# gmlwns2000/sea-attention

Measured on AMD Instinct MI355X. Metric: tokens/sec + achieved HBM GB/s, OPT-1.3B SEA T=4096 k=64, 1/2/4/8 MI355X, higher is better.
Workload: dtype bf16

## Files before the change

sea-attention_amd/csrc/sea_topk.hip:

```cpp
#include "sea_common.hpp"
#include "sea_tail.hpp"
#include "sea_convfrag.hpp"


#ifdef SEA_STAMP
__device__ unsigned long long sea_dbg[16];
#define STAMP(i) do { if (threadIdx.x == 0) { unsigned long long _t = __builtin_amdgcn_s_memtime(); \
  atomicAdd(&sea_dbg[i], _t - _tprev); _tprev = _t; } } while (0)
#else
#define STAMP(i) do {} while (0)
#endif

namespace sea {

constexpr int TK_THREADS = 256;
constexpr int TK_WAVES = TK_THREADS / WAVE;
constexpr int TK_MAX_BINS = 2048;

__device__ inline uint32_t f2key(float f) {
  f = f + 0.0f;
  uint32_t u = __float_as_uint(f);
  return u ^ ((u >> 31) ? 0xFFFFFFFFu : 0x80000000u);
}

struct TopkParams {
  const void* src;
  int64_t sn, sh, st;
  int H, T_dst, T_m, T_src;
  int is_causal, max_k;
  int M;
  int nchunks;
  int W;
  int G;
  const int32_t* keep;
  int64_t keep_stride_n;
  uint32_t* bits;
  float* mask_out;
  int32_t* row_nnz;
  int32_t* head_off;
  const int32_t* t_src_dev;
  int t_src_stride;
  int32_t* crow1;
};

template <typename T> __device__ inline void load4(const T* p, float* f);
template <> __device__ inline void load4<float>(const float* p, float* f) {
  float4 v = *reinterpret_cast<const float4*>(p);
  f[0] = v.x; f[1] = v.y; f[2] = v.z; f[3] = v.w;
}
template <> __device__ inline void load4<__hip_bfloat16>(const __hip_bfloat16* p, float* f) {
  uint2 v = *reinterpret_cast<const uint2*>(p);
  f[0] = __uint_as_float(v.x << 16); f[1] = __uint_as_float(v.x & 0xffff0000u);
  f[2] = __uint_as_float(v.y << 16); f[3] = __uint_as_float(v.y & 0xffff0000u);
}
template <> __device__ inline void load4<__half>(const __half* p, float* f) {
  uint2 v = *reinterpret_cast<const uint2*>(p);
  const __half2* h = reinterpret_cast<const __half2*>(&v);
  float2 a = __half22float2(h[0]), b = __half22float2(h[1]);
  f[0] = a.x; f[1] = a.y; f[2] = b.x; f[3] = b.y;
}

__device__ inline int block_excl_scan(int v, int* s_wave , int* total) {
  const int lane = threadIdx.x & 63, w = threadIdx.x >> 6;
  int incl = wave_incl_scan(v);
  if (lane == 63) s_wave[w] = incl;
  __syncthreads();
  int base = 0, tot = 0;
#pragma unroll
  for (int i = 0; i < TK_WAVES; ++i) {
    int x = s_wave[i];
    if (i < w) base += x;
    tot += x;
  }
  __syncthreads();
  *total = tot;
  return base + incl - v;
}

template <typename T>
__device__ __noinline__ unsigned long long select_multipass(const T* base, int64_t sh, int T_m, int nchunks, int M, int K,
                                                            uint32_t umin, uint32_t umax, int rounds, int* s_hist,
                                                            int* s_wave, int* s_bcast) {
  const int tid = threadIdx.x;
  auto load_keys = [&](int j, uint32_t* k4) -> bool {
    const int c = j * TK_THREADS + tid;
    if (c >= nchunks) { k4[0] = k4[1] = k4[2] = k4[3] = 0u; return false; }
    const int f0 = c * 4;
    const int h = f0 / T_m, b0 = f0 - h * T_m;
    float f[4];
    load4<T>(base + h * sh + b0, f);
    for (int e = 0; e < 4; ++e) k4[e] = f2key(f[e]);
    return true;
  };
  unsigned long long sel = 0;
  uint32_t prefix = umax;
  int bits_left = (umax == umin) ? 0 : (32 - __clz(umax ^ umin));
  int kth = K, n_eq = M;
  while (bits_left > 0) {
    const int d = bits_left < 11 ? bits_left : 11;
    const int shift = bits_left - d;
    const int nb = 1 << d;
    const int hi = shift + d;
    for (int i = tid; i < nb; i += TK_THREADS) s_hist[i] = 0;
    __syncthreads();
    for (int j = 0; j < rounds; ++j) {
      uint32_t k4[4];
      if (!load_keys(j, k4)) continue;
      for (int e = 0; e < 4; ++e) {
        const uint32_t u = k4[e];
        const bool cand = (hi >= 32) ? true : ((u >> hi) == (prefix >> hi));
        if (cand) atomicAdd(&s_hist[nb - 1 - (int)((u >> shift) & (uint32_t)(nb - 1))], 1);
      }
    }
    __syncthreads();
    const int per = (nb + TK_THREADS - 1) / TK_THREADS;
    int mine = 0;
    for (int i = 0; i < per; ++i) {
      const int bi = tid * per + i;
      if (bi < nb) mine += s_hist[bi];
    }
    int total;
    const int excl = block_excl_scan(mine, s_wave, &total);
    if (excl < kth && kth <= excl + mine) {
      int run = excl;
      for (int i = 0; i < per; ++i) {
        const int bi = tid * per + i;
        const int c = s_hist[bi];
        if (kth <= run + c) { s_bcast[0] = bi; s_bcast[1] = run; s_bcast[2] = c; break; }
        run += c;
      }
    }
    __syncthreads();
    const int rb = s_bcast[0];
    kth -= s_bcast[1];
    n_eq = s_bcast[2];
    const uint32_t dmask = (uint32_t)(nb - 1) << shift;
    prefix = (prefix & ~dmask) | ((uint32_t)(nb - 1 - rb) << shift);
    bits_left = shift;
    __syncthreads();
  }
  const uint32_t tau = prefix;
  const int r = kth;
  int seen = 0;
  for (int j = 0; j < rounds; ++j) {
    uint32_t k4[4];
    const bool valid = load_keys(j, k4);
    int cnt = 0;
    for (int e = 0; e < 4; ++e) cnt += (valid && k4[e] == tau) ? 1 : 0;
    int total = 0, rank = 0;
    if (n_eq != r) rank = seen + block_excl_scan(cnt, s_wave, &total);
    for (int e = 0; e < 4; ++e) {
      if (!valid) continue;
      if (k4[e] > tau) sel |= 1ull << (4 * j + e);
      if (k4[e] == tau) {
        if (n_eq == r || rank < r) sel |= 1ull << (4 * j + e);
        ++rank;
      }
    }
    seen += total;
  }
  return sel;
}

__device__ inline long long block_excl_scan64(long long v, long long* s_wave , long long* total) {
  const int lane = threadIdx.x & 63, w = threadIdx.x >> 6;
  long long incl = wave_incl_scan(v);
  if (lane == 63) s_wave[w] = incl;
  __syncthreads();
  long long base = 0, tot = 0;
#pragma unroll
  for (int i = 0; i < TK_WAVES; ++i) {
    const long long x = s_wave[i];
    if (i < w) base += x;
    tot += x;
  }
  __syncthreads();
  *total = tot;
  return base + incl - v;
}

template <typename T, int EPT, bool FROM_MASK, bool FULL, int HMAX = 1024, bool EXT_CAND = false, bool K16 = false, bool HCW = K16>
__device__ __forceinline__ void select_body(const TopkParams& p, uint32_t (&key)[K16 ? EPT / 2 : EPT], unsigned long long sel, int n,
                                            int t, int row, const T* base, uint32_t* cand = nullptr) {
  constexpr int R = EPT / 4;
  static_assert(!K16 || (sizeof(T) == 2 && !FROM_MASK), "packed keys: 16-bit maps");
  auto key_at = [&](int i) -> uint32_t {
    if constexpr (K16) return (i & 1) ? (key[i >> 1] >> 16) : (key[i >> 1] & 0xffffu);
    else return key[i];
  };
  auto digit_at = [&](int i, int shift, int d) -> int {
    if constexpr (K16) return (int)__builtin_amdgcn_ubfe(~key[i >> 1], shift + 16 * (i & 1), d);
    else return (int)__builtin_amdgcn_ubfe(~key[i], shift, d);
  };
  __shared__ int s_hist[TK_MAX_BINS + 1];
  __shared__ int s_head[HMAX];
  __shared__ int s_wave[TK_WAVES];
  __shared__ uint32_t s_red[2 * TK_WAVES];
  __shared__ int s_bcast[4];
  uint32_t* s_ckey;
  uint32_t* s_cidx;
  if constexpr (EXT_CAND) {
    s_ckey = cand; s_cidx = cand + TK_CAND_CAP;
  } else {
    __shared__ uint32_t s_cand[2 * TK_CAND_CAP];
    s_ckey = s_cand; s_cidx = s_cand + TK_CAND_CAP;
  }
  __shared__ uint32_t s_selbits[512];
  __shared__ int s_ncand;

  const int tid = threadIdx.x;
  const int lane = tid & 63, wv = tid >> 6;
#ifdef SEA_STAMP
  unsigned long long _tprev = __builtin_amdgcn_s_memtime();
#endif
  for (int i = tid; i <= TK_MAX_BINS; i += TK_THREADS) s_hist[i] = 0;
  for (int i = tid; i < 512; i += TK_THREADS) s_selbits[i] = 0;
  for (int i = tid; i < p.H; i += TK_THREADS) s_head[i] = 0;
  if (tid == 0) s_ncand = 0;

  if (!FROM_MASK) {
    const int K = p.keep[n * p.keep_stride_n + t + (p.t_src_dev ? p.t_src_dev[n * p.t_src_stride] - p.T_dst : 0)];
    if (K >= p.M) {
#pragma unroll
      for (int j = 0; j < R; ++j)
        if (FULL || j * TK_THREADS + tid < p.nchunks) sel |= 0xFull << (4 * j);
      __syncthreads();
    } else if (K <= 0) {
      __syncthreads();
    } else {
      uint32_t umin = 0xFFFFFFFFu, umax = 0u;
      if constexpr (K16) {
        typedef unsigned short us2 __attribute__((ext_vector_type(2)));
        us2 mn = us2{0xFFFF, 0xFFFF}, mx = us2{0, 0};
#pragma unroll
        for (int j = 0; j < R; ++j) {
          if (FULL || j * TK_THREADS + tid < p.nchunks) {
            const us2 a = __builtin_bit_cast(us2, key[2 * j]), b = __builtin_bit_cast(us2, key[2 * j + 1]);
            mn = __builtin_elementwise_min(mn, __builtin_elementwise_min(a, b));
            mx = __builtin_elementwise_max(mx, __builtin_elementwise_max(a, b));
          }
        }
        umin = min((uint32_t)mn[0], (uint32_t)mn[1]);
        umax = max((uint32_t)mx[0], (uint32_t)mx[1]);
      } else {
#pragma unroll
      for (int j = 0; j < R; ++j) {
        if (FULL || j * TK_THREADS + tid < p.nchunks) {
          umin = min(umin, min(min(key[4 * j], key[4 * j + 1]), min(key[4 * j + 2], key[4 * j + 3])));
          umax = max(umax, max(max(key[4 * j], key[4 * j + 1]), max(key[4 * j + 2], key[4 * j + 3])));
        }
      }
      }
      umin = wave_min(umin);
      umax = wave_max(umax);
      if (lane == 0) { s_red[wv] = umin; s_red[TK_WAVES + wv] = umax; }
      __syncthreads();
#pragma unroll
      for (int i = 0; i < TK_WAVES; ++i) { umin = min(umin, s_red[i]); umax = max(umax, s_red[TK_WAVES + i]); }
      STAMP(1);
      const int bits_left = (umax == umin) ? 0 : (32 - __clz(umax ^ umin));
      bool fast = bits_left > 0;
      int rb_sel = 0, kth = K, c_in = 0, shift = 0, d = 0;
      if (fast) {
        d = bits_left < 11 ? bits_left : 11;
        shift = bits_left - d;
        const int nb = 1 << d;
#pragma unroll
        for (int i = 0; i < EPT; ++i) {
          int rb = digit_at(i, shift, d);
          if (!FULL) rb = (((i >> 2) * TK_THREADS + tid) < p.nchunks) ? rb : TK_MAX_BINS;
          atomicAdd(&s_hist[rb], 1);
        }
        __syncthreads();
        const int per = (nb + TK_THREADS - 1) / TK_THREADS;
        int mine = 0;
        for (int i = 0; i < per; ++i) {
          const int bi = tid * per + i;
          if (bi < nb) mine += s_hist[bi];
        }
        int total;
        const int excl = block_excl_scan(mine, s_wave, &total);
        if (excl < K && K <= excl + mine) {
          int run = excl;
          for (int i = 0; i < per; ++i) {
            const int bi = tid * per + i;
            const int c = s_hist[bi];
            if (K <= run + c) { s_bcast[0] = bi; s_bcast[1] = run; s_bcast[2] = c; break; }
            run += c;
          }
        }
        __syncthreads();
        rb_sel = s_bcast[0];
        kth = K - s_bcast[1];
        c_in = s_bcast[2];
        fast = c_in <= TK_CAND_CAP;
      }
      STAMP(2);
      if (fast) {
#pragma unroll
        for (int i = 0; i < EPT; ++i) {
          const int rb = digit_at(i, shift, d);
          const bool valid = FULL || (((i >> 2) * TK_THREADS + tid) < p.nchunks);
          if (valid && rb < rb_sel) sel |= 1ull << i;
          if (valid && rb == rb_sel) {
            const int slot = atomicAdd(&s_ncand, 1);
            s_ckey[slot] = key_at(i);
            s_cidx[slot] = (uint32_t)(((i >> 2) * TK_THREADS + tid) * 4 + (i & 3));
          }
        }
        __syncthreads();
        for (int ci = tid; ci < c_in; ci += TK_THREADS) {
          const uint32_t ku = s_ckey[ci], kf = s_cidx[ci];
          int rank = 0;
          for (int cj = 0; cj < c_in; ++cj) {
            const uint32_t ou = s_ckey[cj], of = s_cidx[cj];
            rank += (ou > ku || (ou == ku && of < kf)) ? 1 : 0;
          }
          if (rank < kth) atomicOr(&s_selbits[kf >> 5], 1u << (kf & 31));
        }
        __syncthreads();
#pragma unroll
        for (int j = 0; j < R; ++j) {
          const int c = j * TK_THREADS + tid;
          const unsigned long long nibx = (s_selbits[(c >> 3) & 511] >> (4 * (c & 7))) & 0xFu;
          sel |= nibx << (4 * j);
        }
      } else if constexpr (K16) {
        const bool hist = bits_left > 0;
        int n_eq = hist ? c_in : p.M;
        uint32_t tau_low = 0u;
        const uint32_t lowmask = hist ? ((1u << shift) - 1u) : 0u;
        auto in_bin = [&](int i) -> bool {
          const bool valid = FULL || (((i >> 2) * TK_THREADS + tid) < p.nchunks);
          return valid && (!hist || digit_at(i, shift, d) == rb_sel);
        };
        if (hist) {
#pragma unroll
          for (int i = 0; i < EPT; ++i) {
            const bool valid = FULL || (((i >> 2) * TK_THREADS + tid) < p.nchunks);
            if (valid && digit_at(i, shift, d) < rb_sel) sel |= 1ull << i;
          }
          if (shift > 0) {
            const int nb2 = 1 << shift;
            __syncthreads();
            if (tid < nb2) s_hist[tid] = 0;
            __syncthreads();
#pragma unroll
            for (int i = 0; i < EPT; ++i)
              if (in_bin(i)) atomicAdd(&s_hist[nb2 - 1 - (int)(key_at(i) & lowmask)], 1);
            __syncthreads();
            const int mine = tid < nb2 ? s_hist[tid] : 0;
            int total;
            const int excl = block_excl_scan(mine, s_wave, &total);
            if (tid < nb2 && excl < kth && kth <= excl + mine) { s_bcast[0] = tid; s_bcast[1] = excl; s_bcast[2] = mine; }
            __syncthreads();
            tau_low = (uint32_t)(nb2 - 1 - s_bcast[0]);
            kth -= s_bcast[1];
            n_eq = s_bcast[2];
#pragma unroll
            for (int i = 0; i < EPT; ++i)
              if (in_bin(i) && (key_at(i) & lowmask) > tau_low) sel |= 1ull << i;
          }
        }
        int seen = 0;
#pragma unroll
        for (int j = 0; j < R; ++j) {
          bool tie[4];
          int cnt = 0;
#pragma unroll
          for (int e = 0; e < 4; ++e) {
            tie[e] = in_bin(4 * j + e) && (key_at(4 * j + e) & lowmask) == tau_low;
            cnt += tie[e] ? 1 : 0;
          }
          int total = 0, rank = 0;
          if (n_eq != kth) rank = seen + block_excl_scan(cnt, s_wave, &total);
#pragma unroll
          for (int e = 0; e < 4; ++e) {
            if (tie[e]) {
              if (n_eq == kth || rank < kth) sel |= 1ull << (4 * j + e);
              ++rank;
            }
          }
          seen += total;
        }
        __syncthreads();
      } else {
        sel = select_multipass<T>(base, p.sh, p.T_m, p.nchunks, p.M, K, umin, umax, R, s_hist, s_wave, s_bcast);
        for (int i = tid; i < p.H; i += TK_THREADS) s_head[i] = 0;
        __syncthreads();
      }
    }
  } else {
    __syncthreads();
  }

  STAMP(3);
  const int w_t = row_width(t, p.T_dst, p.t_src_dev ? p.t_src_dev[n * p.t_src_stride] : p.T_src, p.is_causal);
  const float scale = interp_scale(w_t, p.T_m);
  const bool tm_pow2 = (p.T_m & (p.T_m - 1)) == 0;
  const int tm_sh = __ffs(p.T_m) - 1;
#pragma unroll
  for (int j = 0; j < R; ++j) {
    const int c = j * TK_THREADS + tid;
    const bool valid = FULL || c < p.nchunks;
    const uint32_t nib = (uint32_t)(sel >> (4 * j)) & 0xFu;
    uint32_t word = nib << (4 * (lane & 7));
    word |= dpp_u32<0xB1>(word);
    word |= dpp_u32<0x4E>(word);
    word |= dpp_u32<0x141>(word);
    if ((lane & 7) == 0 && (c >> 3) < p.W) p.bits[(int64_t)row * p.W + (c >> 3)] = word;
    if (p.mask_out != nullptr && valid) {
      const int f0 = c * 4;
      const int h = f0 / p.T_m, b0 = f0 - h * p.T_m;
      float4 m;
      m.x = (nib & 1u) ? 1.f : 0.f; m.y = (nib & 2u) ? 1.f : 0.f;
      m.z = (nib & 4u) ? 1.f : 0.f; m.w = (nib & 8u) ? 1.f : 0.f;
      *reinterpret_cast<float4*>(p.mask_out + (((int64_t)n * p.H + h) * p.T_dst + t) * p.T_m + b0) = m;
    }
  }
  if constexpr (K16 && HCW) {
    int wpx[4];
    {
      float bprev = interp_bound(4 * lane, scale);
#pragma unroll
      for (int e = 0; e < 4; ++e) {
        const float bnext = interp_bound(4 * lane + e + 1, scale);
        const int w = (int)(bnext - bprev);
        wpx[e] = w < p.max_k ? w : p.max_k;
        bprev = bnext;
      }
    }
#pragma unroll
    for (int j0 = 0; j0 < R; j0 += 8) {
      float red[8];
#pragma unroll
      for (int b = 0; b < 8; ++b) {
        int sum = 0;
        if (j0 + b < R) {
          const uint32_t nib = (uint32_t)(sel >> (4 * (j0 + b))) & 0xFu;
#pragma unroll
          for (int e = 0; e < 4; ++e) sum += (nib >> e) & 1u ? wpx[e] : 0;
        }
        red[b] = (float)sum;
      }
      const float x = wave_reduce8(red, [](float u, float v) { return u + v; });
#pragma unroll
      for (int b = 0; b < 8; ++b) {
        const int h = 4 * (j0 + b) + wv;
        if (j0 + b < R && h < p.H && lane == 0) s_head[h] = (int)reduce8_get(x, b);
      }
    }
  } else {
    unsigned long long m = sel;
    while (m) {
      const int i = __ffsll((long long)m) - 1;
      m &= m - 1;
      const int f = ((i >> 2) * TK_THREADS + tid) * 4 + (i & 3);
      const int h = tm_pow2 ? (f >> tm_sh) : f / p.T_m, b = f - h * p.T_m;
      int w = (int)(interp_bound(b + 1, scale) - interp_bound(b, scale));
      w = w < p.max_k ? w : p.max_k;
      if (w > 0) atomicAdd(&s_head[h], w);
    }
  }
  __syncthreads();
  STAMP(4);
  if (wv == 0) {
    int carry = 0;
    int32_t* ho = p.head_off + (int64_t)row * (p.H + 1);
    for (int h0 = 0; h0 < p.H; h0 += 64) {
      const int h = h0 + lane;
      const int v = h < p.H ? s_head[h] : 0;
      const int incl = wave_incl_scan(v);
      if (h < p.H) ho[h] = carry + incl - v;
      carry += __shfl(incl, 63);
    }
    if (lane == 0) {
      ho[p.H] = carry; p.row_nnz[row] = carry;
      if (p.crow1 != nullptr) { p.crow1[2 * row] = 0; p.crow1[2 * row + 1] = carry; }
    }
  }
}

template <typename T, int EPT, bool FROM_MASK, bool FULL>
__global__ __launch_bounds__(TK_THREADS) void topk_select_kernel(TopkParams p) {
  constexpr int R = EPT / 4;
  const int tid = threadIdx.x;
  const int row = blockIdx.x;
  const int n = row / p.T_dst, t = row - n * p.T_dst;
  const T* base = reinterpret_cast<const T*>(p.src) + n * p.sn + t * p.st;
#ifdef SEA_STAMP
  unsigned long long _tprev = __builtin_amdgcn_s_memtime();
#endif

  uint32_t key[EPT];
  unsigned long long sel = 0;
#pragma unroll
  for (int j = 0; j < R; ++j) {
    const int c = j * TK_THREADS + tid;
    float f[4] = {0.f, 0.f, 0.f, 0.f};
    const bool valid = FULL || c < p.nchunks;
    if (valid) {
      const int f0 = c * 4;
      const int h = f0 / p.T_m, b0 = f0 - h * p.T_m;
      load4<T>(base + h * p.sh + b0, f);
    }
#pragma unroll
    for (int e = 0; e < 4; ++e) {
      if (FROM_MASK) {
        if (valid && f[e] != 0.f) sel |= 1ull << (4 * j + e);
        key[4 * j + e] = 0;
      } else {
        key[4 * j + e] = valid ? f2key(f[e]) : 0u;
      }
    }
  }
  STAMP(0);
  select_body<T, EPT, FROM_MASK, FULL>(p, key, sel, n, t, row, base);
}

template <typename T, int EPT, bool FULL>
__device__ __forceinline__ void tail_select_row(const TailParams& tp, const TopkParams& p, float* s_z, int row) {
#include "sea_tail_select_row.inc"
}

template <typename T, int EPT, bool FULL>
#ifndef SEA_TSEL_OCC32
#define SEA_TSEL_OCC32 7
#endif
#ifndef SEA_TSEL_OCC16
#define SEA_TSEL_OCC16 7
#endif
__global__ __launch_bounds__(TK_THREADS, EPT <= 16 ? SEA_TSEL_OCC16 : EPT == 32 ? SEA_TSEL_OCC32 : EPT == 40 ? 5 : 1) void predictor_tail_select_kernel(TailParams tp, TopkParams p) {
  extern __shared__ __attribute__((aligned(16))) float s_z[];
  const int row = blockIdx.x;
#include "sea_tail_select_row.inc"
}

template <int EPT>
__global__ __launch_bounds__(TK_THREADS) void predictor_tail_select_f32_kernel(TailParams tp, TopkParams p) {
  using T = float;
  constexpr bool FULL = false;
  static_assert(EPT <= 32, "one batch of eight heads per wave (H <= 32)");
  extern __shared__ __attribute__((aligned(16))) float s_z[];
  const int row = blockIdx.x;
#include "sea_tail_select_row.inc"
}

template <typename T, int E, int EPT>
__device__ __forceinline__ void tail_select_row_gen(const TailParams& tp, const TopkParams& p, float* s_z, int row) {
  constexpr bool TAB_LDS = false;
#include "sea_tail_select_row_gen.inc"
}

template <typename T, int E, int EPT>
__global__ __launch_bounds__(TK_THREADS) void predictor_tail_select_gen_kernel(TailParams tp, TopkParams p) {
  constexpr bool TAB_LDS = true;
  extern __shared__ __attribute__((aligned(16))) float s_z[];
  const int row = blockIdx.x;
#include "sea_tail_select_row_gen.inc"
}

template <typename I>
__global__ __launch_bounds__(1024) void row_scan_kernel(const int32_t* row_nnz, int T_dst, I* crow) {
  constexpr int PER = 16;
  __shared__ int s_w[2][16];
  const int n = blockIdx.x;
  const int tid = threadIdx.x, lane = tid & 63, w = tid >> 6;
  const int32_t* src = row_nnz + (int64_t)n * T_dst;
  I* dst = crow + (int64_t)n * (T_dst + 1);
  long long carry = 0;
  for (int t0 = 0; t0 < T_dst; t0 += 1024 * PER) {
    int vv[PER];
#pragma unroll
    for (int j = 0; j < PER; ++j) {
      const int t = t0 + j * 1024 + tid;
      vv[j] = t < T_dst ? src[t] : 0;
    }
#pragma unroll
    for (int j = 0; j < PER; ++j) {
      if (t0 + j * 1024 < T_dst) {
        const int t = t0 + j * 1024 + tid;
        const int v = vv[j];
        const int incl = wave_incl_scan(v);
        if (lane == 63) s_w[j & 1][w] = incl;
        __syncthreads();
        int base = 0, tot = 0;
#pragma unroll
        for (int i = 0; i < 16; ++i) { const int x = s_w[j & 1][i]; if (i < w) base += x; tot += x; }
        if (t < T_dst) dst[t] = (I)(carry + base + incl - v);
        carry += tot;
      }
    }
    __syncthreads();
  }
  if (tid == 0) dst[T_dst] = (I)carry;
}

struct EmitParams {
  const uint32_t* bits;
  const void* crow;
  int H, T_dst, T_m, T_src, is_causal, max_k, W;
  void* col;
  int64_t col_stride_n, z_cap;
  float* values_out;
  int T_enc;
  const int32_t* t_src_dev;
  int t_src_stride;
};

constexpr int EM_TABLE = 1024;
constexpr int EM_WIN = 4096;

template <typename I>
__device__ __forceinline__ void csr_emit_row(const EmitParams& p, const int row) {
  __shared__ int s_wave[TK_WAVES];
  __shared__ int s_bound[EM_TABLE + 1];
  __shared__ int s_out[EM_WIN];
  const int tid = threadIdx.x;
  const int n = row / p.T_dst, t = row - n * p.T_dst;
  const I* crow = reinterpret_cast<const I*>(p.crow) + (int64_t)n * (p.T_dst + 1);
  const int64_t row_beg = (int64_t)crow[t];
  const int64_t row_end = (int64_t)crow[t + 1];
  if (row_end == row_beg) return;
  I* col = reinterpret_cast<I*>(p.col) + n * p.col_stride_n;
  float* vals = p.values_out ? p.values_out + n * p.col_stride_n : nullptr;
  const uint32_t* bits = p.bits + (int64_t)row * p.W;
  const int w_t = row_width(t, p.T_dst, p.t_src_dev ? p.t_src_dev[n * p.t_src_stride] : p.T_src, p.is_causal);
  const float scale = interp_scale(w_t, p.T_m);
  const bool table = p.T_m <= EM_TABLE;
  if (table)
    for (int m = tid; m <= p.T_m; m += TK_THREADS) s_bound[m] = (int)interp_bound(m, scale);
  __syncthreads();
  auto bnd = [&](int m) { return table ? s_bound[m] : (int)interp_bound(m, scale); };
  const bool aligned = (p.T_m & 31) == 0;
  const bool direct = sizeof(I) == 4 && vals == nullptr && aligned && w_t >= 4 * p.T_m && (w_t + p.T_m - 1) / p.T_m <= p.max_k;

  int carry = 0;
  for (int w0 = 0; w0 < p.W; w0 += TK_THREADS) {
    const int wi = w0 + tid;
    uint32_t word = wi < p.W ? bits[wi] : 0u;
    const int f0 = wi * 32;
    const int h0 = f0 / p.T_m, b0 = f0 - h0 * p.T_m;
    int nent = 0;
    if (direct) {
      const int npmax = __builtin_amdgcn_readfirstlane(wave_max(__popc(word)));
      uint32_t m = word;
      for (int it = 0; it < npmax; ++it) {
        const bool act = m != 0u;
        const int b = b0 + (act ? __ffs(m) - 1 : 0);
        m &= m - 1;
        const int wd = bnd(b + 1) - bnd(b);
        nent += act ? wd : 0;
      }
    } else {
      for (uint32_t m = word; m;) {
        const int bit = __ffs(m) - 1;
        m &= m - 1;
        int b = b0 + bit;
        if (!aligned) b %= p.T_m;
        const int wd = bnd(b + 1) - bnd(b);
        nent += wd < p.max_k ? wd : p.max_k;
      }
    }
    int total;
    const int excl = block_excl_scan(nent, s_wave, &total);
    if (direct) {
      const int wlo = w_t / p.T_m;
      const int nst = (wlo + 1 + 3) >> 2;
      const int npmax = __builtin_amdgcn_readfirstlane(wave_max(__popc(word)));
      int64_t off = row_beg + carry + excl;
      uint32_t m = word;
      const int hb = h0 * p.T_enc;
      for (int it = 0; it < npmax; ++it) {
        const bool act = m != 0u;
        const int bit = act ? __ffs(m) - 1 : 0;
        m &= m - 1;
        const int b = b0 + bit;
        const int lo = bnd(b), hi = bnd(b + 1);
        const int wd = hi - lo;
        if (act && off + wd <= p.z_cap) {
          int32_t* dst = reinterpret_cast<int32_t*>(col) + off;
          const int c0 = hb + hi - 1;
          typedef int ei4 __attribute__((ext_vector_type(4), aligned(4)));
          for (int i = 0; i < nst; ++i) {
            const int j = min(4 * i, wd - 4);
            const int c = c0 - j;
            const ei4 v = {c, c - 1, c - 2, c - 3};
            *reinterpret_cast<ei4*>(dst + j) = v;
          }
        }
        off += act ? wd : 0;
      }
      carry += total;
      continue;
    }
    for (int win = (carry / EM_WIN) * EM_WIN; win < carry + total; win += EM_WIN) {
      int off = carry + excl;
      if (nent > 0 && off < win + EM_WIN && off + nent > win) {
        const bool inside = off >= win && off + nent <= win + EM_WIN;
        for (uint32_t m = word; m;) {
          const int bit = __ffs(m) - 1;
          m &= m - 1;
          int h = h0, b = b0 + bit;
          if (!aligned) { const int q = b / p.T_m; h += q; b -= q * p.T_m; }
          const int lo = bnd(b), hi = bnd(b + 1);
          const int wd = hi - lo;
          const int hb = h * p.T_enc;
          if (wd <= p.max_k) {
            if (inside) {
              int* dst = s_out + (off - win);
              const int c0 = hb + hi - 1;
              for (int j = 0; j < wd; ++j) dst[j] = c0 - j;
            } else {
              for (int j = 0; j < wd; ++j) {
                const int o = off + j - win;
                if ((unsigned)o < (unsigned)EM_WIN) s_out[o] = hb + hi - 1 - j;
              }
            }
            off += wd;
          } else {
// ... 661 lines not shown
```

Before: 16.30 million.

## Classify top-k candidates with scalar key-range compares and wave-aggregated slot allocation

The fast top-k path used to extract a radix digit per element and take one shared-memory atomicAdd for each candidate. It now compares each key against a wave-uniform key range held in SGPRs using inline v_cmp/v_addc asm, which builds 'above' and 'candidate' bitmasks directly. It then reserves candidate slots with one atomic per wave via a wave prefix scan, and uses a binary select tree to read keys out of the register array. The bitmask store loop is also split so all words are computed first and stored afterwards. The inline asm and the key-range derivation from umax add correctness risk across edge cases.

```diff
diff --git a/sea-attention_amd/csrc/sea_topk.hip b/sea-attention_amd/csrc/sea_topk.hip
--- a/sea-attention_amd/csrc/sea_topk.hip
+++ b/sea-attention_amd/csrc/sea_topk.hip
@@ -179,6 +179,23 @@
   return base + incl - v;
 }
 
+__device__ __forceinline__ void shift_in_gt_ge(uint32_t& a, uint32_t& b, uint32_t top, uint32_t lo, uint32_t x) {
+  asm("v_cmp_lt_u32_e32 vcc, %2, %4\n\tv_addc_co_u32_e32 %0, vcc, %0, %0, vcc\n\t"
+      "v_cmp_le_u32_e32 vcc, %3, %4\n\tv_addc_co_u32_e32 %1, vcc, %1, %1, vcc"
+      : "+v"(a), "+v"(b) : "s"(top), "s"(lo), "v"(x) : "vcc");
+}
+
+template <int LO, int N, int NK> __device__ __forceinline__ uint32_t pick_reg(const uint32_t (&a)[NK], int r) {
+  static_assert(N >= 1 && LO + N <= NK, "inside the array");
+  if constexpr (N == 1) {
+    return a[LO];
+  } else {
+    constexpr int HALF = 1 << (31 - __builtin_clz((unsigned)(N - 1)));
+    const uint32_t lo = pick_reg<LO, HALF>(a, r), hi = pick_reg<LO + HALF, N - HALF>(a, r);
+    return (r & HALF) ? hi : lo;
+  }
+}
+
 template <typename T, int EPT, bool FROM_MASK, bool FULL, int HMAX = 1024, bool EXT_CAND = false, bool K16 = false, bool HCW = K16>
 __device__ __forceinline__ void select_body(const TopkParams& p, uint32_t (&key)[K16 ? EPT / 2 : EPT], unsigned long long sel, int n,
                                             int t, int row, const T* base, uint32_t* cand = nullptr) {
@@ -297,17 +314,62 @@
       }
       STAMP(2);
       if (fast) {
-#pragma unroll
-        for (int i = 0; i < EPT; ++i) {
-          const int rb = digit_at(i, shift, d);
-          const bool valid = FULL || (((i >> 2) * TK_THREADS + tid) < p.nchunks);
-          if (valid && rb < rb_sel) sel |= 1ull << i;
-          if (valid && rb == rb_sel) {
-            const int slot = atomicAdd(&s_ncand, 1);
-            s_ckey[slot] = key_at(i);
-            s_cidx[slot] = (uint32_t)(((i >> 2) * TK_THREADS + tid) * 4 + (i & 3));
+        constexpr int NW = (EPT + 31) / 32;
+        constexpr int KSH = K16 ? 16 : 0;
+        const uint32_t nbm = (1u << d) - 1u;
+        const uint32_t lo_k = (((umax >> shift) & ~nbm) | (nbm - (uint32_t)rb_sel)) << shift;
+        const uint32_t top_k = lo_k | ((1u << shift) - 1u);
+        uint32_t bin_lo = __builtin_amdgcn_readfirstlane(lo_k << KSH);
+        uint32_t bin_top = __builtin_amdgcn_readfirstlane((top_k << KSH) | (K16 ? 0xffffu : 0u));
+        asm volatile("s_nop 1" : "+s"(bin_lo), "+s"(bin_top));
+        const int nvalid = FULL ? R : (p.nchunks - tid + TK_THREADS - 1) / TK_THREADS;
+        uint32_t candw[NW];
+        int ncl = 0;
+#pragma unroll
+        for (int w = 0; w < NW; ++w) {
+          constexpr int NE_MAX = 32;
+          const int ne = EPT - 32 * w < NE_MAX ? EPT - 32 * w : NE_MAX;
+          uint32_t above = 0u, notbelow = 0u;
+#pragma unroll
+          for (int e = NE_MAX - 1; e >= 0; --e) {
+            if (e >= ne) continue;
+            const int i = 32 * w + e;
+            uint32_t x;
+            if constexpr (K16) x = (i & 1) ? key[i >> 1] : key[i >> 1] << 16;
+            else x = key[i];
+            shift_in_gt_ge(above, notbelow, bin_top, bin_lo, x);
           }
-        }
+          if (!FULL) {
+            const int nv = nvalid - 8 * w;
+            const uint32_t vm = nv >= 8 ? 0xFFFFFFFFu : nv <= 0 ? 0u : (1u << (4 * nv)) - 1u;
+            above &= vm;
+            notbelow &= vm;
+          }
+          const uint32_t cnd = notbelow & ~above;
+          sel |= (unsigned long long)above << (32 * w);
+          candw[w] = cnd;
+          ncl += __popc(cnd);
+        }
+        const int incl = wave_incl_scan(ncl);
+        const int wtot = __builtin_amdgcn_readlane(incl, 63);
+        int slot = 0;
+        if (wtot != 0) {
+          if (lane == 63) slot = atomicAdd(&s_ncand, wtot);
+          slot = __builtin_amdgcn_readlane(slot, 63);
+        }
+        slot += incl - ncl;
+#pragma unroll
+        for (int w = 0; w < NW; ++w) {
+          for (uint32_t m = candw[w]; m != 0u; m &= m - 1u) {
+            const int e = __ffs(m) - 1;
+            uint32_t ku = pick_reg<0, K16 ? EPT / 2 : EPT>(key, K16 ? 16 * w + (e >> 1) : 32 * w + e);
+            if constexpr (K16) ku = (ku >> (16 * (e & 1))) & 0xffffu;
+            s_ckey[slot] = ku;
+            s_cidx[slot] = (uint32_t)((((32 * w + e) >> 2) * TK_THREADS + tid) * 4 + (e & 3));
+            ++slot;
+          }
+        }
+        STAMP(6);
         __syncthreads();
         for (int ci = tid; ci < c_in; ci += TK_THREADS) {
           const uint32_t ku = s_ckey[ci], kf = s_cidx[ci];
@@ -399,23 +461,34 @@
   const float scale = interp_scale(w_t, p.T_m);
   const bool tm_pow2 = (p.T_m & (p.T_m - 1)) == 0;
   const int tm_sh = __ffs(p.T_m) - 1;
+  uint32_t word[R];
 #pragma unroll
   for (int j = 0; j < R; ++j) {
-    const int c = j * TK_THREADS + tid;
-    const bool valid = FULL || c < p.nchunks;
-    const uint32_t nib = (uint32_t)(sel >> (4 * j)) & 0xFu;
-    uint32_t word = nib << (4 * (lane & 7));
-    word |= dpp_u32<0xB1>(word);
-    word |= dpp_u32<0x4E>(word);
-    word |= dpp_u32<0x141>(word);
-    if ((lane & 7) == 0 && (c >> 3) < p.W) p.bits[(int64_t)row * p.W + (c >> 3)] = word;
-    if (p.mask_out != nullptr && valid) {
-      const int f0 = c * 4;
-      const int h = f0 / p.T_m, b0 = f0 - h * p.T_m;
-      float4 m;
-      m.x = (nib & 1u) ? 1.f : 0.f; m.y = (nib & 2u) ? 1.f : 0.f;
-      m.z = (nib & 4u) ? 1.f : 0.f; m.w = (nib & 8u) ? 1.f : 0.f;
-      *reinterpret_cast<float4*>(p.mask_out + (((int64_t)n * p.H + h) * p.T_dst + t) * p.T_m + b0) = m;
+    uint32_t wd = ((uint32_t)(sel >> (4 * j)) & 0xFu) << (4 * (lane & 7));
+    wd |= dpp_u32<0xB1>(wd);
+    wd |= dpp_u32<0x4E>(wd);
+    wd |= dpp_u32<0x141>(wd);
+    word[j] = wd;
+  }
+  if ((lane & 7) == 0) {
+    uint32_t* bw = p.bits + (int64_t)row * p.W + (tid >> 3);
+#pragma unroll
+    for (int j = 0; j < R; ++j)
+      if (FULL || j * (TK_THREADS / 8) + (tid >> 3) < p.W) bw[j * (TK_THREADS / 8)] = word[j];
+  }
+  if (p.mask_out != nullptr) {
+#pragma unroll
+    for (int j = 0; j < R; ++j) {
+      const int c = j * TK_THREADS + tid;
+      if (FULL || c < p.nchunks) {
+        const uint32_t nib = (uint32_t)(sel >> (4 * j)) & 0xFu;
+        const int f0 = c * 4;
+        const int h = f0 / p.T_m, b0 = f0 - h * p.T_m;
+        float4 m;
+        m.x = (nib & 1u) ? 1.f : 0.f; m.y = (nib & 2u) ? 1.f : 0.f;
+        m.z = (nib & 4u) ? 1.f : 0.f; m.w = (nib & 8u) ? 1.f : 0.f;
+        *reinterpret_cast<float4*>(p.mask_out + (((int64_t)n * p.H + h) * p.T_dst + t) * p.T_m + b0) = m;
+      }
     }
   }
   if constexpr (K16 && HCW) {
```

Measured after the change: 16.32 million, median of 5. Within noise of the previous version (+0.1%).
